# lh3/bwa

Hardware: AMD Instinct MI355X
Metric: Mreads/s (whole job) 2x150 bp vs GRCh38-scale index; SAM bit-identical to bwa mem (gate: `parity`).  `value` = the hot path (mem_align1_core of every read) on batches resident in HBM, as the bench contract times it; the SAM-producing FASTQ->SAM rate of the same build is `end_to_end_pe.value` (also i (higher is better)
Workload: dtype int32/u64 (integer DP + FM-index ranks); 1 GPU; 500000 pairs of 2x150 bp (mates interleaved) per GPU per step vs seeded synthetic 3100 Mbp genome (GRCh38 stand-in, seq_len 6.2e+09; BASELINE configs[2] layout); reads_per_gpu=1000000, read_len=150, layout=pe, sa_intv=1, occ_block_bytes=32, batches_in_flight=3

## Files before the change

bwa_amd/api.py:

```python
from __future__ import annotations

import ctypes as C
import os

import numpy as np

try:
    import torch
except Exception:
    torch = None

from .structs import ALN_DTYPE, ALNREG_DTYPE, PAIR_DTYPE, PESTAT_DTYPE, PESTAT_INFO_DTYPE, PRIMARY_DTYPE, RESCUE_DTYPE, SAMPE_DTYPE, MemOpt, PeOut, SamIn, SamOut

HERE = os.path.dirname(os.path.abspath(__file__))
DEFAULT_LIB = os.path.join(HERE, "csrc", "libbwagpu.so")

INTV3_DTYPE = np.dtype([("x0", "<u8"), ("x2", "<u8"), ("info", "<u8")])
GCHAIN_DTYPE = np.dtype([("n_seeds", "<i4"), ("rid", "<i4"), ("w", "<i4"), ("kept", "<i4"), ("is_alt", "<i4"),
                         ("frac_rep", "<f4"), ("pos", "<i8")])
GSEED_DTYPE = np.dtype([("rbeg", "<i8"), ("qbeg", "<i4"), ("len", "<i4"), ("score", "<i4"), ("_pad", "<i4")])
assert GCHAIN_DTYPE.itemsize == 32 and GSEED_DTYPE.itemsize == 24


MATESW_DTYPE = np.dtype([("read", "<i4"), ("r", "<i4"), ("anchor_rb", "<i8"), ("anchor_rid", "<i4"), ("score", "<i4"), ("te", "<i4"), ("qe", "<i4"),
# ... 7 lines not shown
SORT_KEY_DTYPE = np.dtype([("a", "<i8"), ("b", "<i4"), ("c", "<i4")])
assert SORT_KEY_DTYPE.itemsize == 16


class Stats(C.Structure):
    _fields_ = [(n, C.c_int64) for n in (
        "n_reads", "n_bases", "n_intv", "n_seeds", "n_chains", "n_regs_raw", "n_regs", "n_occ_blocks", "n_lf_steps",
        "n_ext_calls", "n_ext_cells", "n_glb_calls", "n_glb_cells", "ref_bases", "n_sw_calls", "n_sw_cells")] + [
        (n, C.c_float) for n in ("ms_seed", "ms_sa", "ms_chain", "ms_seedsw", "ms_extend", "ms_dedup", "ms_total")] + [
        ("n_retries", C.c_int32), ("ms_publish", C.c_float), ("n_tab_lookups", C.c_int64), ("n_bt_nodes", C.c_int64), ("n_chain_recs", C.c_int64),
        ("n_chain_deferred", C.c_int64), ("n_ext_fast", C.c_int64), ("n_chain_deferred2", C.c_int64),
        ("ms_pack", C.c_float), ("ms_download_copy", C.c_float), ("ms_cigar_kernels", C.c_float), ("ms_cigar_copy", C.c_float),
        ("n_cig_cells", C.c_int64), ("n_cig_dp", C.c_int64), ("retry_mask", C.c_int32), ("reserved_", C.c_int32)]

    def as_dict(self):
        return {n: getattr(self, n) for n, _ in self._fields_ if n != "reserved_"}


EXPORTS = [
    "bwagpu_create", "bwagpu_create_from_files", "bwagpu_destroy", "bwagpu_strerror", "bwagpu_last_error", "bwagpu_version",
    "bwagpu_index_info", "bwagpu_densify_sa", "bwagpu_set_stats", "bwagpu_get_stats", "bwagpu_align_bseq", "bwagpu_align_flat",
    "bwagpu_free", "bwagpu_batch_upload", "bwagpu_batch_run", "bwagpu_batch_download", "bwagpu_set_taps", "bwagpu_tap_intervals",
    "bwagpu_tap_chains", "bwagpu_tap_regs_raw", "bwagpu_index_buffers", "bwagpu_index_export", "bwagpu_clone", "bwagpu_index_ready",
    "bwagpu_batch_cigars", "bwagpu_batch_cigar_ops", "bwagpu_debug_phase", "bwagpu_batch_matesw", "bwagpu_clone_to_device", "bwagpu_index_build", "bwagpu_built_free", "bwagpu_abi_sizes", "bwagpu_debug_prof", "bwagpu_debug_hist", "bwagpu_debug_seed_x2", "bwagpu_debug_chain_hist", "bwagpu_debug_dp", "bwagpu_debug_sort", "bwagpu_debug_sort_limits", "bwagpu_set_cigar_filter", "bwagpu_batch_reserve", "bwagpu_batch_footprint", "bwagpu_mem_info",
    "bwagpu_batch_primary", "bwagpu_primary_flat", "bwagpu_primary_limits", "bwagpu_batch_pair", "bwagpu_pair_flat", "bwagpu_pair_limits", "bwagpu_batch_rescue", "bwagpu_rescue_flat", "bwagpu_rescue_limits",
    "bwagpu_batch_pestat", "bwagpu_pestat_flat", "bwagpu_batch_pestat_hist", "bwagpu_pestat_finish", "bwagpu_pestat_limits",
    "bwagpu_batch_alns", "bwagpu_alns_flat", "bwagpu_alns_limits", "bwagpu_aln_size",
    "bwagpu_cigars_flat", "bwagpu_cigar_limits", "bwagpu_dedup_flat", "bwagpu_dedup_limits", "bwagpu_ext_limits", "bwagpu_seed_limits",
    "bwagpu_batch_sampe", "bwagpu_sampe_flat", "bwagpu_sampe_limits", "bwagpu_sampe_size",
    "bwagpu_set_contig_names", "bwagpu_batch_sam", "bwagpu_sam_flat", "bwagpu_sam_limits",
    "bwagpu_trim", "bwagpu_set_option", "bwagpu_get_option", "bwagpu_set_default_option", "bwagpu_clear_default_options", "bwagpu_option_name",
]


class IndexDesc(C.Structure):
    _fields_ = [("bwt", C.c_void_p), ("bwt_size", C.c_uint64), ("primary", C.c_uint64), ("L2", C.c_uint64 * 5), ("seq_len", C.c_uint64),
                ("sa", C.c_void_p), ("n_sa", C.c_uint64), ("sa_intv", C.c_int), ("pac", C.c_void_p), ("l_pac", C.c_int64),
                ("n_seqs", C.c_int32), ("ctg_offset", C.c_void_p), ("ctg_len", C.c_void_p), ("ctg_is_alt", C.c_void_p)]


class BwaGpuError(RuntimeError):
    pass


def load_library(path: str | None = None) -> C.CDLL:
    path = path or DEFAULT_LIB
    if not os.path.exists(path):
# ... 763 lines not shown
```

bwa_amd/csrc/bwagpu.hip:

```cpp
#include <hip/hip_runtime.h>
#include <stdio.h>
#include <stdlib.h>
#include <string.h>
#include <math.h>
#include <algorithm>
#include <atomic>
#include <map>
#include <memory>
#include <mutex>
#include <string>
#include <vector>
#include <chrono>

#include "bwagpu_config.h"
#include "dev_common.h"
#include "dev_fm.h"
#include "dev_sort.h"
#include "dev_seed.h"
#include "dev_chain.h"
#include "dev_chainw.h"
#include "dev_ext.h"
#include "dev_extw.h"
#include "dev_extp.h"
#include "dev_dedup.h"
// ... 187 lines not shown
{
	if (b.ensure(bytes ? bytes : 16)) { h->err = "hipMalloc failed"; return BWAGPU_ENOMEM; }
	if (bytes) HIPCHK(h, hipMemcpy(b.p, src, bytes, hipMemcpyHostToDevice));
	return 0;
}

namespace {
std::mutex g_cfg_m;
std::map<std::string, long long> g_cfg_defaults;
}
static bool option_in_range(const BwagpuConfig &c, const long long *f, long long value)
{
	auto in = [&](long long lo, long long hi) { return value >= lo && value <= hi; };
	if (f == &c.ext_occ) return value == 4 || value == 6;
	if (f == &c.seed_mrg) return value == -1 || value == 0 || value == 2;
	if (f == &c.share) return in(-1, 100);
	if (f == &c.seed_task_stack || f == &c.seed_p2_cap || f == &c.mem_cap || f == &c.seed_grid || f == &c.cig_ops_cap || f == &c.idx_desc_max_mb || f == &c.pri_log_cap || f == &c.pair_tab_cap) return in(0, 0x3fffffff);
	if (f == &c.seed_budget || f == &c.dedup_heavy) return in(-1, 0x3fffffff);
	if (f == &c.dedup_stage || f == &c.dedup_big || f == &c.dedup_net) return in(-1, 1024);
	if (f == &c.seed_lds_ent) return in(-1, 16);
	if (f == &c.dedup_ring) return value == 0 || (in(256, 4096) && (value & (value - 1)) == 0);
	if (f == &c.cigl_mib) return in(0, 1 << 20);
	if (f == &c.cig_tiers || f == &c.chain_regs) return in(0, 2);
	if (f == &c.chain_flt_lds) return in(0, CW_FLT_LDS);
	if (f == &c.ptab_m) return in(0, PTAB_MAX);
	if (f == &c.occ32_sb_shift) return in(8, 32);
	return true;
}
static void init_config(BwagpuConfig &c)
{
	c = BwagpuConfig();
	const BwagpuConfig dflt;
	c.from_env();
#define X(name, d) if (!option_in_range(c, &c.name, c.name)) { fprintf(stderr, "[W::bwagpu] BWAGPU_%s=%lld is out of range: ignored\n", #name, c.name); c.name = dflt.name; }
	BWAGPU_OPTION_LIST(X)
#undef X
	std::lock_guard<std::mutex> l(g_cfg_m);
	for (auto &kv : g_cfg_defaults) if (long long *f = c.field(kv.first.c_str())) *f = kv.second;
	g_results.on = c.pinned_results; g_results.min_kb = c.pinned_min_kb < 0 ? 0 : c.pinned_min_kb; g_results.cap_mb = c.pinned_cap_mb < 0 ? 0 : c.pinned_cap_mb; g_results.inited = true;
}
extern "C" int bwagpu_set_default_option(const char *key, long long value)
{
	BwagpuConfig probe;
	const long long *f = probe.field(key);
	if (!f || !option_in_range(probe, f, value)) return BWAGPU_EINVAL;
	std::lock_guard<std::mutex> l(g_cfg_m);
// ... 37 lines not shown
__global__ void __launch_bounds__(256) k_ptab_level(DevIndex ix, u64 *tab, int j)
{
	const u64 n = (u64)1 << (2 * j);
	for (u64 c = (u64)blockIdx.x * blockDim.x + threadIdx.x; c < n; c += (u64)gridDim.x * blockDim.x) {
		BiIntv out;
		if (j == 1) fm_init(ix, (int)c, out);
		else {
			const u64 *pe = tab + ((((u64)1 << (2 * (j - 1))) - 4) / 3 + (c >> 2)) * 3;
			BiIntv par; par.x0 = pe[0]; par.x1 = pe[1]; par.x2 = pe[2]; par.info = 0;
			fm_extend1(ix, par, 3 - (int)(c & 3), 0, out);
		}
		u64 *e = tab + ((n - 4) / 3 + c) * 3;
		e[0] = out.x0; e[1] = out.x1; e[2] = out.x2;
	}
}

__global__ void __launch_bounds__(256) k_ptab_records(const u64 *tab, uint4 *rec, int m)
{
	const u64 n = ((u64)1 << (2 * m)) * (u64)m;
	for (u64 t = (u64)blockIdx.x * blockDim.x + threadIdx.x; t < n; t += (u64)gridDim.x * blockDim.x) {
		const u64 w = t / (u64)m; const int j = (int)(t % (u64)m) + 1;
		const u64 *e = tab + ((((u64)1 << (2 * j)) - 4) / 3 + (w >> (2 * (m - j)))) * 3;
		BiIntv v; v.x0 = e[0]; v.x1 = e[1]; v.x2 = e[2]; v.info = 0;
		rec[t] = SeedStack::pack(v);
	}
}

DEVFN void occ32_start_counts(const DevIndex &ix, u64 j, u64 cnt[4])
{
	const uint4 *src = ix.bwt + (j >> 1) * 4;
	const uint4 c01 = src[0], c23 = src[1];
	cnt[0] = (u64)c01.y << 32 | c01.x; cnt[1] = (u64)c01.w << 32 | c01.z; cnt[2] = (u64)c23.y << 32 | c23.x; cnt[3] = (u64)c23.w << 32 | c23.z;
	if (j & 1) {
		const uint4 w0 = src[2];
		u32 c1 = 0, c2 = 0, c3 = 0;
		count_pair(w0.x, w0.y, 32, c1, c2, c3); count_pair(w0.z, w0.w, 32, c1, c2, c3);
		cnt[0] += 64 - c1 - c2 - c3; cnt[1] += c1; cnt[2] += c2; cnt[3] += c3;
	}
}
__global__ void __launch_bounds__(256) k_occ32_sb(DevIndex ix, u64 *sb, u64 n_sb, u64 n_new, int sh )
{
	for (u64 s = (u64)blockIdx.x * blockDim.x + threadIdx.x; s < n_sb; s += (u64)gridDim.x * blockDim.x) {
		u64 cnt[4] = { 0, 0, 0, 0 };
		if ((s << sh) < n_new) occ32_start_counts(ix, s << sh, cnt);
		for (int k = 0; k < 4; ++k) sb[s * 4 + k] = cnt[k];
	}
// ... 345 lines not shown
	if (ctg_is_alt) memcpy(ctg_is_alt, h->h_ctg_alt.data(), (size_t)h->n_seqs * 4);
	return BWAGPU_OK;
}

extern "C" int bwagpu_index_info(const bwagpu_t *h, int64_t *l_pac, int32_t *n_seqs, uint64_t *seq_len, int *sa_intv)
{
	if (!h) return BWAGPU_EINVAL;
	if (l_pac) *l_pac = h->l_pac;
	if (n_seqs) *n_seqs = h->n_seqs;
	if (seq_len) *seq_len = h->seq_len;
	if (sa_intv) *sa_intv = h->sa_intv;
	return BWAGPU_OK;
}

extern "C" int bwagpu_debug_phase(const bwagpu_t *h) { return h ? h->phase : -1; }
extern "C" int bwagpu_debug_prof(bwagpu_t *h, unsigned long long out[16])
{
	if (!h || !out || !h->d_ctr.p) return BWAGPU_EINVAL;
	Counters c;
	if (hipMemcpy(&c, h->d_ctr.p, sizeof c, hipMemcpyDeviceToHost) != hipSuccess) return BWAGPU_EHIP;
	for (int i = 0; i < 16; ++i) out[i] = c.prof[i];
	out[8] = c.n_vr_ovf + c.prof[8];
	out[0] = c.n_heavy; out[1] = c.n_p2_tasks;
	return BWAGPU_OK;
}

extern "C" int bwagpu_debug_seed_x2(bwagpu_t *h, unsigned long long out[8])
{
	if (!h || !out || !h->d_ctr.p) return BWAGPU_EINVAL;
	Counters c;
	if (hipMemcpy(&c, h->d_ctr.p, sizeof c, hipMemcpyDeviceToHost) != hipSuccess) return BWAGPU_EHIP;
	for (int i = 0; i < 8; ++i) out[i] = c.seed_x2[i];
	return BWAGPU_OK;
}
extern "C" int bwagpu_debug_hist(bwagpu_t *h, unsigned long long out[256])
{
	if (!h || !out || !h->d_ctr.p) return BWAGPU_EINVAL;
	Counters c;
	if (hipMemcpy(&c, h->d_ctr.p, sizeof c, hipMemcpyDeviceToHost) != hipSuccess) return BWAGPU_EHIP;
	for (int i = 0; i < 64; ++i) out[i] = c.seed_hist[i];
	for (int i = 0; i < 96; ++i) { out[64 + i] = c.wave_hist[0][i]; out[160 + i] = c.wave_hist[1][i]; }
	return BWAGPU_OK;
}
extern "C" int bwagpu_debug_chain_hist(bwagpu_t *h, unsigned long long out[192])
{
	if (!h || !out || !h->d_ctr.p) return BWAGPU_EINVAL;
// ... 360 lines not shown
		Batch B; memset(&B, 0, sizeof B);
		B.n_reads = n; B.max_len = h->max_len; B.stats = h->stats_on;
		B.seq = h->d_seq.as<u8>(); B.seq_nib = h->d_seq_nib.as<u64>(); B.off = h->d_off.as<i64>(); B.ctr = h->d_ctr.as<Counters>();
		B.tmp_intv = h->d_tmp_intv.as<BiIntv>(); B.mem_cap = h->mem_cap;
		B.rd_words = h->rd_words; B.seq_2b = h->d_seq_2b.as<u32>(); B.seq_flags = h->d_seq_flags.as<u8>();
		const int lane_lds = SEED_LANE_LDS, ent_max = SEED_LDS_ENT;
		const int lds_ent_dflt = h->rd_words ? ((lane_lds - 4 * h->rd_words) / 16 < ent_max ? (lane_lds - 4 * h->rd_words) / 16 : ent_max) : ent_max;
		B.seed_lds_ent = (h->seq_len < ((u64)1 << 37) && h->max_len < 65536) ? (cfg.seed_lds_ent >= 0 ? (int)cfg.seed_lds_ent : lds_ent_dflt) : 0;
		h->seed_lds_run = B.seed_lds_ent;
		if (((size_t)(B.seed_lds_ent ? B.seed_lds_ent : 1) * 16 + (size_t)B.rd_words * 4) * BLOCK > 65536) B.rd_words = 0;
		B.intv_n = h->d_intv_n.as<i32>(); B.intv_off = h->d_intv_off.as<i64>(); B.intv = h->d_intv.as<Intv3>();
		B.seed_n = h->d_seed_n.as<i32>(); B.seed_off = h->d_seed_off.as<i64>(); B.slot_cap = h->slot_cap;
		B.slot_pos = h->d_slot_pos.as<u64>(); B.slot_qbeg = h->d_slot_qbeg.as<i32>(); B.slot_len = h->d_slot_len.as<i32>(); B.slot_rid = h->d_slot_rid.as<i32>(); B.slot_blob = h->d_slot_blob.as<u8>();
		B.chain_n = h->d_chain_n.as<i32>(); B.node_off = h->d_node_off.as<i64>(); B.nodes = h->d_nodes.as<i32>(); B.node_cap = h->node_cap;
		B.reg_off = h->d_reg_off.as<i64>(); B.reg_cap_r = h->d_reg_cap_r.as<i32>(); B.reg_n_raw = h->d_reg_n_raw.as<i32>(); B.reg_n = h->d_reg_n.as<i32>();
		B.regs = h->d_regs.as<bwagpu_alnreg_t>(); B.reg_cap = h->reg_cap;
		B.regs_raw = h->taps_on ? h->d_regs_raw.as<bwagpu_alnreg_t>() : nullptr;
		B.dp_h = h->d_dp_h.as<i32>(); B.dp_e = h->d_dp_e.as<i32>(); B.dp_waves = dp_wave_count(h, n_threads);
		B.seedsw_minhsp = h->d_minhsp.as<i32>();
		B.order = h->d_order.as<i32>(); B.bin_cnt = h->d_bin_cnt.as<u32>(); B.seed_w = h->d_seed_w.as<i32>(); B.seed_order = nullptr;
		B.seed_prio = cfg.seed_prio != 0;
		B.ext_blk = cfg.ext_blk != 0;
		B.seed_no_virt = cfg.seed_no_virt != 0;
		B.seed_pass3_inline = cfg.seed_pass3_inline != 0;
		B.task_step = opt->min_seed_len; B.n_vreads = n_vreads; B.vr_ovf_run = 0; B.vr_room = 0; B.seed_stack_cap = 0; B.intv_n3 = nullptr;
		if (seed_tasks) { B.vr_first = h->d_vr_tab.as<i32>(); B.vr_ovf = h->d_vr_ovf.as<i32>(); B.intv_n3 = h->d_intv_n3.as<i32>(); }
		B.task_tpr = 0; B.p2_tasks = nullptr; B.p2_cap = 0; B.heavy_list = nullptr; B.seed_budget = 0;
		if (heavy_tasks) {
			const i64 p2_cap = cfg.seed_p2_cap > 0 ? cfg.seed_p2_cap * (i64)h->p2_factor : (i64)((double)n * .5 * h->p2_factor) + 4096;
			B.heavy_list = h->d_heavy.as<i32>(); B.seed_budget = seed_budget;
			if (h->d_p2_tasks.ensure((size_t)p2_cap * 8)) { h->err = "hipMalloc failed (seeding tasks)"; return BWAGPU_ENOMEM; }
			B.intv_n3 = h->d_intv_n3.as<i32>(); B.p2_tasks = h->d_p2_tasks.as<i64>(); B.p2_cap = p2_cap;
		}
		int seed_mrg = (cfg.seed_mrg >= 0 ? cfg.seed_mrg : 2) ? 2 : 0;
		if (!idx_in_desc) seed_mrg = 0;
		B.seq_nib_bytes = (((u64)h->n_bases + 15) / 16) * 8;
		dim3 grid(n_threads / BLOCK), block(BLOCK);
		HIPCHK(h, hipEventRecord(h->ev[0], h->stream));
		if (dbg_sync) { hipError_t e_ = hipStreamSynchronize(h->stream); fprintf(stderr, "[bwagpu] attempt %d: %s done (%s)\n", attempt, "start", hipGetErrorString(e_)); }
		if (!B.seed_pass3_inline) {
			if (h->ix.occ32 != nullptr && seed_mrg) hipLaunchKernelGGL((k_seed3<1, true>), grid, block, 0, h->stream, h->ix, *opt, B);
			else if (h->ix.occ32 != nullptr) hipLaunchKernelGGL(k_seed3<1>, grid, block, 0, h->stream, h->ix, *opt, B);
			else hipLaunchKernelGGL(k_seed3<0>, grid, block, 0, h->stream, h->ix, *opt, B);
			if (!cfg.seed_input_order) {
				i32 *keep = B.order; B.order = h->d_seed_order.as<i32>();
				if (int rc2 = order_reads(h, B, B.seed_w)) return rc2;
// ... 2070 lines not shown
```

bwa_amd/csrc/bwagpu_config.h:

```cpp
#pragma once
#include <stdlib.h>
#include <string.h>
#include <ctype.h>
#include <string>

#define BWAGPU_OPTION_LIST(X) \
	X(occ32,             1)     \
	X(occ32_sb_shift,    32)    \
	X(ptab_m,            10)    \
	X(idx_desc_max_mb,   0)     \
	X(seed_mrg,          -1)    \
	X(seed_tasks,        -1)    \
	X(seed_budget,       -1)    \
	X(seed_p2_cap,       0)     \
	X(seed_task_stack,   0)     \
	X(publish_blk,       -1)    \
	X(seedsw_lds,        -1)    \
	X(dedup_blk,         -1)    \
	X(seed_lds_ent,      -1)    \
	X(seed_rd_lds,       1)     \
	X(seed_no_virt,      0)     \
	X(seed_prio,         1)     \
	X(seed_input_order,  0)     \
	X(seed_pass3_inline, 0)     \
	X(seed_grid,         0)     \
	X(share,             -1)    \
	X(ext_pack,          0)     \
	X(ext_blk,           -1)    \
	X(ext_occ,           6)     \
	X(chain_regs,        2)     \
	X(chain_flt_lds,     256)   \
	X(dedup_heavy,       -1)    \
	X(dedup_stage,       -1)    \
	X(dedup_big,         -1)    \
	X(dedup_net,         -1)    \
	X(dedup_prio,        1)     \
	X(dedup_wave,        0)     \
	X(dedup_ring,        0)     \
	X(mem_cap,           0)     \
	X(cig_tiers,         2)     \
	X(cig_ops_cap,       0)     \
	X(cig_long,          1)     \
	X(cigl_mib,          32768) \
	X(pri_log_cap,       0)     \
// ... 29 lines not shown
```

bwa_amd/csrc/dev_common.h:

```cpp
#pragma once
#include <hip/hip_runtime.h>
#include <stdint.h>
#include "../../include/bwagpu.h"

typedef uint64_t u64;
typedef int64_t i64;
typedef uint32_t u32;
typedef int32_t i32;
typedef uint8_t u8;

#define DEVFN __device__ __forceinline__
#ifndef DEV_KEEP
#define DEV_KEEP(v) asm volatile("" : "+v"(v))
#endif
typedef __amdgpu_buffer_rsrc_t BufRsrc;

struct DevIndex {
	const uint4 *bwt;
	u64 primary, L2[5], seq_len;
	const u64 *sa;
	u64 sa_mask;
	int sa_shift;
	const u8 *pac;
	i64 l_pac;
// ... 93 lines not shown
	RegionView v;
	v.chain = (ChainRec*)b; v.kinfo = (int4*)(b + (size_t)64 * n); v.cchain = (bwagpu_chain_t*)(b + (size_t)80 * n);
	v.cseed = (bwagpu_seed_t*)(b + (size_t)112 * n); v.srt = (u64*)(b + (size_t)136 * n);
	v.next = (i32*)(b + (size_t)144 * n); v.ord = (i32*)(b + (size_t)148 * n); v.kept = (i32*)(b + (size_t)152 * n);
	return v;
}

struct Batch {
	int n_reads;
	int max_len;
	int stats;
	const u8 *seq;
	u64 *seq_nib;
	u64 seq_nib_bytes;
	const i64 *off;
	u32 *seq_2b;
	u8 *seq_flags;
	int rd_words;
	Counters *ctr;
	BiIntv *tmp_intv;
	int seed_stack_cap;
	int seed_lds_ent;
	int seed_no_virt;
	int mem_cap;
	i32 *seed_w;
	const i32 *seed_order;
	i32 *intv_n;
	i64 *intv_off;
	Intv3 *intv;
	i32 *seed_n;
	i64 *seed_off;
	i64 slot_cap;
	u64 *slot_pos;
	i32 *slot_qbeg, *slot_len;
	i32 *slot_rid;
	u8 *slot_blob;
	i32 *chain_n;
	int task_step, n_vreads;
	int task_tpr;
	i32 *heavy_list;
	i32 *dd_list;
	int dd_heavy_min, dd_stage_cap;
	int dd_net;
	int dd_prio;
	i32 *dd_form;
	int seed_budget;
// ... 40 lines not shown
```

bwa_amd/csrc/dev_seed.h:

```cpp
#pragma once
#include "dev_fm.h"
#include "dev_sort.h"

#define PTAB_MAX 12
#define SEED_CAND_BITS 64

struct SeedEmit {
	Intv3 *intv; int r, n, cap; bool overflow;
	int min_seed_len;
	i32 *shared_n;
	DEVFN Intv3 *mem() const { return intv + (size_t)r * (size_t)cap; }
	int split_len, base; u64 split_width, cand;
	DEVFN void add(u64 x0, u64 x2, int start, int end) {
		if (end - start < min_seed_len) return;
		Intv3 v; v.x0 = x0; v.x2 = x2; v.info = (u64)start << 32 | (u32)end;
		if (shared_n) {
			const int k = atomicAdd(&shared_n[r], 1);
			if (k >= cap) overflow = true; else mem()[k] = v;
			return;
		}
		if (n == cap) { overflow = true; return; }
		if (end - start >= split_len && x2 <= split_width && n - base < SEED_CAND_BITS) cand |= 1ull << (n - base);
		mem()[n++] = v;
	}
// ... 13 lines not shown
	const u32 *rd;
	int rd_on;
	const u8 *raw; const i64 *off;
	u64 min_intv, last_x2;
	int sx, i, n0, nprev, nc, j, c, ret, last_start;
	int lo;
	bool any;
	BiIntv ik;
	u32 code;
	u32 smask, srem, snew;
	int ncl;
	int top;
	int slot;
	SeedEmit em;
};

struct SeedStack {
	uint4 *lds_base;
	BiIntv *glob_base; int glob_cap;
	DEVFN uint4 *lds_col() const { return lds_base + threadIdx.x; }
	DEVFN BiIntv *glob_col() const { return glob_base + (size_t)(blockIdx.x * blockDim.x + threadIdx.x) * (size_t)glob_cap + PTAB_MAX; }
	int stride, n_lds;
	int virt_m;
	DEVFN void push_fw(SeedLane &L, const BiIntv &v) const {
		const int len = (int)v.info - L.sx;
		if (len < virt_m) L.smask |= 1u << (len - 1); else push(L, v);
	}
	static DEVFN uint4 pack(const BiIntv &v) {
		uint4 w;
		w.x = (u32)v.x0; w.y = (u32)v.x1; w.z = (u32)v.x2;
		w.w = (u32)(v.x0 >> 32) | (u32)(v.x1 >> 32) << 5 | (u32)(v.x2 >> 32) << 10 | (u32)v.info << 16;
		return w;
	}
	static DEVFN BiIntv unpack(const uint4 &w) {
		BiIntv v;
		v.x0 = (u64)(w.w & 31) << 32 | w.x; v.x1 = (u64)(w.w >> 5 & 31) << 32 | w.y; v.x2 = (u64)(w.w >> 10 & 31) << 32 | w.z;
		v.info = w.w >> 16;
		return v;
	}
	DEVFN void push(SeedLane &L, const BiIntv &v) const {
		if (n_lds == 0) glob_col()[L.n0] = v;
		else {
			if (L.n0 >= n_lds) ((uint4*)glob_col())[L.n0 - n_lds] = lds_col()[L.slot * stride];
			lds_col()[L.slot * stride] = pack(v);
			L.slot = L.slot + 1 == n_lds ? 0 : L.slot + 1;
		}
// ... 39 lines not shown
		for (int k = 0; k < 4; ++k)
			for (int b = 0; b < 4; ++b) {
				u32 c = d[k] >> (8 * b) & 255;
				o |= (u64)(c > 3 ? 4 : c) << ((k * 4 + b) * 4);
			}
		B.seq_nib[w] = o;
	}
}

__global__ void __launch_bounds__(256) k_pack_reads2b(Batch B)
{
	const u64 total = (u64)B.n_reads * (u64)B.rd_words;
	for (u64 t = (u64)blockIdx.x * blockDim.x + threadIdx.x; t < total; t += (u64)gridDim.x * blockDim.x) {
		const int r = (int)(t / (u32)B.rd_words), j = (int)(t % (u32)B.rd_words);
		const i64 b0 = B.off[r] + 16 * (i64)j, left = B.off[r + 1] - b0;
		u32 o = 0; bool any_n = false;
		for (int k = 0; k < 16 && k < left; ++k) {
			const u32 c = B.seq[b0 + k];
			if (c > 3) any_n = true; else o |= c << (2 * k);
		}
		B.seq_2b[t] = o;
		if (any_n) B.seq_flags[r] = 1;
	}
}

DEVFN void smem_finish(SeedLane &L) { if (L.pass == 1) { L.x = L.ret; L.st = SS_PASS1; } else L.st = SS_PASS2; }

DEVFN void bwd_begin_row(SeedLane &L, const SeedStack &S, const u64 *nib, int m)
{
	for (;;) {
		if (L.i < L.lo) { smem_finish(L); return; }
		L.c = L.i < 0 ? -1 : seed_q(L, nib, L.i);
		if (L.c > 3) L.c = -1;
		L.j = 0; L.nc = 0; L.ncl = 0; L.last_x2 = 0; L.srem = L.smask; L.snew = 0;
		if (L.c >= 0) { if (m > 0) L.code = (u32)L.c << (2 * (m - 1)) | L.code >> 2; L.st = SS_BWD; return; }
		if (!L.any || L.i + 1 < L.last_start) {
			if (L.nprev > 0) { BiIntv p = S.load(L, 0); L.em.add(p.x0, p.x2, L.i + 1, (int)p.info); }
			L.any = true; L.last_start = L.i + 1;
		}
		smem_finish(L);
		return;
	}
}

DEVFN void fwd_finish(SeedLane &L, const SeedStack &S, const u64 *nib, int m)
{
// ... 8 lines not shown
{
	out = SeedStack::unpack(ix.ptab[(u64)w * (u32)ix.ptab_m + (u32)(j - 1)]);
}

struct SeedBufs { Occ32Bufs occ; BufRsrc ptab, stk, nib; };
template <bool WIN = false> DEVFN int ext_one_trip(const DevIndex &ix, const SeedBufs &bf, bool ext, bool blocks, const BiIntv &src, int c, int back, int tl, u32 code, BiIntv &ok, u32 pf_off, uint4 &pf, u32 win_off = BUF_OOB, u64 *win = nullptr)
{
	const Occ32Pos pp = occ32_pos(ix, src, back);
	Occ32Data od;
	uint4 te = buf_load16(bf.ptab, ext && !blocks ? (code * (u32)ix.ptab_m + (u32)(tl - 1)) << 4 : BUF_OOB);
	occ32_issue(ix, bf.occ, blocks, pp, c, od);
	pf = buf_load16(bf.stk, pf_off);
	uint2 wv = make_uint2(0, 0);
	if (WIN) { wv = buf_load8(bf.nib, win_off); DEV_KEEP(wv.x); DEV_KEEP(wv.y); *win = (u64)wv.y << 32 | wv.x; }
	occ32_keep(od); dev_keep(te); dev_keep(pf);
	int nb = 0;
	if (ext) {
		if (!blocks) ok = SeedStack::unpack(te);
		else nb = occ32_finish(ix, src, c, back, pp, od, ok);
	}
	return nb;
}

DEVFN u32 window_code(SeedLane &L, const u64 *nib, int x, int m)
{
	u32 rc = 0;
	for (int k = 0; k < m; ++k) { const int g = x + k; rc = rc << 2 | (u32)((g < L.len ? seed_q(L, nib, g) : 0) & 3); }
	return rc;
}


DEVFN void smem_start(const DevIndex &ix, SeedLane &L, const SeedStack &S, const u64 *nib, int x, u64 min_intv, int pass)
{
	L.pass = pass; L.sx = x; L.min_intv = min_intv < 1 ? 1 : min_intv;
	const int c0 = seed_q(L, nib, x);
	if (c0 > 3) { L.ret = x + 1; smem_finish(L); return; }
	fm_init(ix, c0, L.ik); L.ik.info = (u64)(x + 1);
	L.i = x + 1; L.n0 = 0; L.slot = 0; L.smask = 0;
	L.code = window_code(L, nib, x, ix.ptab_m);
	if (L.i >= L.len || seed_q(L, nib, L.i) > 3) {
		S.push_fw(L, L.ik); L.ret = (int)L.ik.info;
		fwd_finish(L, S, nib, ix.ptab_m);
	} else L.st = SS_FWD;
}

__global__ void __launch_bounds__(256) k_publish(bwagpu_opt_t opt, Batch B)
{
	u64 nintv = 0;
	for (int r = blockIdx.x * blockDim.x + threadIdx.x; r < B.n_reads; r += gridDim.x * blockDim.x) {
		int n = B.intv_n[r];
		if (n > B.mem_cap) { atomicOr(&B.ctr->overflow, 16ull); B.intv_n[r] = 0; n = 0; }
		B.intv_off[r] = (i64)r * B.mem_cap;
		B.seed_n[r] = 0; B.seed_off[r] = 0; B.node_off[r] = 0;
		if (n == 0) continue;
		Intv3 *iv = B.intv + (size_t)r * B.mem_cap;
		dev_introsort(iv, n, IntvInfoLess());
		i64 ns = 0;
		for (int i = 0; i < n; ++i) {
			const u64 x2 = iv[i].x2;
			u64 step = x2 > (u64)opt.max_occ ? x2 / opt.max_occ : 1;
			u64 cnt = (x2 + step - 1) / step;
			ns += (i64)(cnt < (u64)opt.max_occ ? cnt : (u64)opt.max_occ);
// ... 111 lines not shown
					i64 k = 0;
					for (u32 c = 0; c < cnt; ++c, k += step, ++s) { B.slot_pos[s] = p.x0 + (u64)k; B.slot_qbeg[s] = qb; B.slot_len[s] = sl; }
				}
				base += (u32)s_bcast[0];
				__syncthreads();
			}
		}
		__syncthreads();
	}
	if (B.stats && tid == 0) atomicAdd(&B.ctr->n_intv, (unsigned long long)nintv);
}

template<bool RD, bool STATS, int BLK, int OCC, int MRG = 0, int LR = 0>
__global__ void __launch_bounds__(256, OCC) k_seed(DevIndex ix, bwagpu_opt_t opt, Batch B)
{
	HIP_DYNAMIC_SHARED(uint4, seed_lds)
	const int cap = B.seed_stack_cap > 0 ? B.seed_stack_cap : B.max_len + 1 + PTAB_MAX;
	const int split_len = (int)(opt.min_seed_len * opt.split_factor + .499);
	SeedLane L;
	SeedStack S;
	S.lds_base = seed_lds; S.stride = blockDim.x; S.n_lds = B.seed_lds_ent;
	S.glob_base = B.tmp_intv; S.glob_cap = cap;
	S.virt_m = (ix.ptab_m >= 2 && opt.min_seed_len > ix.ptab_m && !B.seed_no_virt) ? ix.ptab_m : 0;
	L.smask = L.srem = L.snew = 0; L.ncl = 0;
	L.em.intv = B.intv; L.em.r = -1; L.em.cap = B.mem_cap; L.em.min_seed_len = opt.min_seed_len;
	L.em.split_len = split_len; L.em.split_width = (u64)opt.split_width; L.em.cand = 0; L.em.base = 0; L.em.shared_n = LR == 1 ? B.intv_n : nullptr;
	L.lo = -1;
	int vr_task = -1, vr_run = 0;
	const unsigned long long n_tasks = LR == 1 ? (B.vr_ovf_run ? B.ctr->n_vr_ovf : B.task_tpr > 0 ? B.ctr->n_heavy * (unsigned long long)B.task_tpr : (unsigned long long)B.n_vreads)
									 : LR == 3 ? (B.ctr->n_p2_tasks < (unsigned long long)B.p2_cap ? B.ctr->n_p2_tasks : (unsigned long long)B.p2_cap) : 0;
	if (LR == 3) L.em.shared_n = B.intv_n;
	int p2_entry = 0;
	L.st = SS_FETCH; L.len = 0; L.qoff = 0; L.win = 0; L.win_w = ~0u; L.win2 = 0; L.win2_w = ~0u;
	u32 *rd_lds = (u32*)(seed_lds + (size_t)(B.seed_lds_ent ? B.seed_lds_ent : 1) * blockDim.x);
	L.rd = rd_lds; L.rd_on = 0; L.raw = B.seq; L.off = B.off;
	const u64 *nib = RD ? nullptr : B.seq_nib;
	u32 nblk = 0, ntab = 0;
	int pool_base = 0, pool_cnt = 0, pool_r = 0;
	int deferred = 0;
	u32 n_iter = 0, n_slow = 0, n_ext_lanes = 0, n_deep = 0, n_deep_l = 0, n_pf_l = 0, n_win_l = 0;
	u32 n_done_l = 0, n_wait_l = 0, n_slowrun_l = 0, n_first_done = 0;
	u32 n_x2[6] = { 0, 0, 0, 0, 0, 0 }; bool run_f = false, run_b = false;
	u32 my_iter = 0;
	uint4 pf = make_uint4(0, 0, 0, 0);
	SeedBufs bf;
	if (MRG && BLK == 1) {
// ... 141 lines not shown
				case SS_PASS3:
					while (L.x < L.len && seed_q(L, nib, L.x) > 3) ++L.x;
					if (L.x >= L.len) L.st = SS_FINAL;
					else {
						const int c0 = seed_q(L, nib, L.x);
						fm_init(ix, c0, L.ik); L.sx = L.x; L.i = L.x + 1;
						L.code = window_code(L, nib, L.x, ix.ptab_m);
						if (L.i >= L.len) { L.x = L.len; }
						else if (seed_q(L, nib, L.i) > 3) { L.x = L.i + 1; }
						else L.st = SS_STRAT;
					}
					break;
				default: break;
				}
			}
		}
		const int st = L.st;
		if (STATS) n_ext_lanes += (u32)__popcll(__ballot(st == SS_FWD || st == SS_BWD || st == SS_STRAT));
		if (STATS && __ballot(st == SS_BWD && L.j >= S.n_lds && L.j < L.nprev)) ++n_deep;
		const bool ext = st == SS_FWD || st == SS_BWD || st == SS_STRAT;
		BiIntv ok, src, p;
		p.x0 = p.x1 = p.x2 = p.info = 0;
		const int back = st == SS_BWD;
		bool short_ent = false;
		int cb = 0, tl = 0;
		ok.x0 = ok.x1 = ok.x2 = ok.info = 0; src = ok;
		if (ext) {
			if (back) {
				if (L.j < L.nprev) {
					if (STATS && L.j >= S.n_lds) { ++n_deep_l; if (MRG == 2 && pf.w != 0) ++n_pf_l; }
					if (MRG == 2 && pf.w != 0) p = SeedStack::unpack(pf); else p = S.load(L, L.j);
				} else {
					const int len = 32 - __clz((int)L.srem);
					L.srem &= ~(1u << (len - 1));
					p.x0 = p.x1 = p.x2 = 0; p.info = (u64)(L.i + 1 + len); short_ent = true;
				}
			}
			src.x0 = back ? p.x0 : L.ik.x0; src.x1 = back ? p.x1 : L.ik.x1; src.x2 = back ? p.x2 : L.ik.x2; src.info = 0;
			const int qi = back ? 0 : seed_q(L, nib, L.i);
			cb = back ? L.c : 3 - qi;
			tl = back ? (int)p.info - L.i : L.i - L.sx + 1;
		}
		const bool blocks = ext && tl > ix.ptab_m;
		if (MRG && BLK == 1) {
			u32 pf_off = BUF_OOB;
			if (MRG == 2 && back && !short_ent && S.n_lds && L.j + 1 < L.nprev && L.j + 1 >= S.n_lds)
				pf_off = ((u32)threadIdx.x * (u32)S.glob_cap + PTAB_MAX) * (u32)sizeof(BiIntv) + (u32)(L.top - (L.j + 1)) * (u32)sizeof(uint4);
			u32 nb;
			if (MRG == 2 && !RD) {
				u32 win_off = BUF_OOB, ww = 0; u64 wnew = 0;
				const int want = back ? L.i - 1 : L.i + 1;
				if (ext && want >= 0 && want < L.len) {
					ww = (u32)((L.qoff + (u64)want) >> 4);
					if (ww != L.win_w && ww != L.win2_w) win_off = ww << 3;
				}
				nb = (u32)ext_one_trip<true>(ix, bf, ext, blocks, src, cb, back, tl, L.code, ok, pf_off, pf, win_off, &wnew);
				if (win_off != BUF_OOB && B.seq_nib_bytes <= BUF_MAX_BYTES) { L.win2 = wnew; L.win2_w = ww; if (STATS) ++n_win_l; }
			} else nb = (u32)ext_one_trip(ix, bf, ext, blocks, src, cb, back, tl, L.code, ok, pf_off, pf);
			if (STATS && ext) { if (blocks) nblk += nb; else ++ntab; }
		}
		if (STATS && ext && blocks) {
			const bool one = src.x2 == 1;
			++n_x2[back ? 1 : 0]; if (one) ++n_x2[back ? 3 : 2];
			if (one && !(back ? run_b : run_f)) ++n_x2[back ? 5 : 4];
			if (back) run_b = one; else run_f = one;
		}
		if (ext) {
			if (MRG && BLK == 1) ;
			else if (!blocks) { ptab_load(ix, tl, L.code, ok); if (STATS) ++ntab; }
			else { const u32 nb = fm_extend1<BLK>(ix, src, cb, back, ok); if (STATS) nblk += nb; }
			if (LR == 1 && st == SS_FWD && L.n0 >= B.vr_room) {
				const unsigned long long k = atomicAdd(&B.ctr->n_vr_ovf, 1ull);
				B.vr_ovf[k] = vr_task;
				L.st = SS_FINAL;
			} else
			if (st == SS_FWD) {
				bool stop = false;
				if (ok.x2 != L.ik.x2) {
					S.push_fw(L, L.ik); L.ret = (int)L.ik.info;
					if (ok.x2 < L.min_intv) stop = true;
				}
				if (!stop) {
					ok.info = (u64)(L.i + 1); L.ik = ok; ++L.i;
					if (L.i >= L.len || seed_q(L, nib, L.i) > 3) { S.push_fw(L, L.ik); L.ret = (int)L.ik.info; stop = true; }
				}
				if (stop) fwd_finish(L, S, nib, ix.ptab_m);
			} else if (st == SS_BWD) {
				if (ok.x2 < L.min_intv) {
					if (L.nc == 0 && (!L.any || L.i + 1 < L.last_start)) {
						L.em.add(p.x0, p.x2, L.i + 1, (int)p.info); L.any = true; L.last_start = L.i + 1;
					}
				} else if (L.nc == 0 || ok.x2 != L.last_x2) {
					ok.info = p.info;
					const int nl = (int)p.info - L.i;
					if (nl < S.virt_m) L.snew |= 1u << (nl - 1);
					else { S.store(L, L.ncl, ok); ++L.ncl; }
					++L.nc; L.last_x2 = ok.x2;
				}
				if (!short_ent) ++L.j;
				if (L.j >= L.nprev && L.srem == 0) {
					if (L.nc == 0) smem_finish(L);
					else { L.nprev = L.ncl; L.smask = L.snew; --L.i; bwd_begin_row(L, S, nib, ix.ptab_m); }
				}
			} else {
				if (ok.x2 < opt.max_mem_intv && L.i - L.sx >= opt.min_seed_len) {
					if (ok.x2 > 0) L.em.add(ok.x0, ok.x2, L.sx, L.i + 1);
					L.x = L.i + 1; L.st = SS_PASS3;
				} else {
					L.ik = ok; ++L.i;
					if (L.i >= L.len) { L.x = L.len; L.st = SS_PASS3; }
					else if (seed_q(L, nib, L.i) > 3) { L.x = L.i + 1; L.st = SS_PASS3; }
				}
			}
		}
	}
	if (STATS) {
		atomicAdd(&B.ctr->occ_blocks, (unsigned long long)nblk); atomicAdd(&B.ctr->tab_lookups, (unsigned long long)ntab);
		for (int k = 0; k < 6; ++k) atomicAdd(&B.ctr->seed_x2[k], (unsigned long long)n_x2[k]);
		atomicAdd(&B.ctr->prof[9], (unsigned long long)n_win_l); atomicAdd(&B.ctr->prof[10], (unsigned long long)n_deep_l); atomicAdd(&B.ctr->prof[11], (unsigned long long)n_pf_l);
		if ((threadIdx.x & 63) == 0) { atomicAdd(&B.ctr->prof[12], (unsigned long long)n_deep); atomicAdd(&B.ctr->prof[13], (unsigned long long)n_iter); atomicAdd(&B.ctr->prof[14], (unsigned long long)n_slow); atomicAdd(&B.ctr->prof[15], (unsigned long long)n_ext_lanes);
// ... 13 lines not shown
		const Intv3 *iv = B.intv + (size_t)r * (size_t)B.mem_cap;
		for (int e = n3; e < n; ++e) {
			const Intv3 p = iv[e];
			const int start = (int)(p.info >> 32), end = (int)(u32)p.info;
			if (end - start < split_len || p.x2 > (u64)opt.split_width) continue;
			const unsigned long long t = atomicAdd(&B.ctr->n_p2_tasks, 1ull);
			if ((long long)t < B.p2_cap) B.p2_tasks[t] = (i64)r << 32 | (u32)e; else atomicOr(&B.ctr->overflow, 32ull);
		}
	}
}

template <int BLK, bool MRG = false> __global__ void __launch_bounds__(256, 3) k_seed3(DevIndex ix, bwagpu_opt_t opt, Batch B)
{
	SeedLane L;
	L.em.cap = B.mem_cap; L.em.min_seed_len = opt.min_seed_len; L.em.intv = B.intv; L.em.r = -1; L.em.n = 0; L.em.overflow = false;
	L.em.split_len = 0x7fffffff; L.em.split_width = 0; L.em.cand = 0; L.em.base = 0; L.em.shared_n = nullptr;
	L.len = 0; L.qoff = 0; L.win = 0; L.win_w = ~0u; L.win2 = 0; L.win2_w = ~0u; L.x = 0; L.sx = 0; L.i = 0; L.code = 0; L.rd = nullptr; L.rd_on = 0; L.raw = nullptr; L.off = nullptr;
	L.ik.x0 = L.ik.x1 = L.ik.x2 = L.ik.info = 0;
	const u64 *nib = B.seq_nib;
	const int lane = threadIdx.x & 63;
	enum { T_FETCH = 0, T_START, T_EXT, T_DONE };
	int st = T_FETCH, pool_base = 0, pool_cnt = 0;
	u32 nblk = 0, ntab = 0, weight = 0;
	SeedBufs bf;
	if (MRG && BLK == 1) { bf.occ = occ32_bufs(ix); bf.ptab = buf_rsrc(ix.ptab, ix.ptab_bytes); bf.stk = buf_rsrc(nullptr, 0); bf.nib = bf.stk; }
	while (__ballot(st != T_DONE)) {
		const u64 wm = __ballot(st == T_FETCH);
		if (wm) {
			if (pool_cnt == 0) {
				const int first = __ffsll((unsigned long long)__ballot(1)) - 1;
				const unsigned long long old = atomicAdd(&B.ctr->next_read3, lane == first ? 64ull : 0ull);
				pool_base = __shfl((int)old, first); pool_cnt = 64;
			}
			const int rank = __popcll(wm & ((1ull << lane) - 1));
			if (st == T_FETCH && rank < pool_cnt) {
				const int r = pool_base + rank;
				if (r >= B.n_reads) st = T_DONE;
				else {
					L.em.r = r; L.qoff = (u64)B.off[r]; L.len = (int)(B.off[r + 1] - B.off[r]);
					L.em.n = 0; L.em.overflow = false;
					B.intv_n[r] = 0; B.seed_w[r] = 0; weight = 0;
					if (B.intv_n3) B.intv_n3[r] = 0;
					if (L.len >= opt.min_seed_len && opt.max_mem_intv > 0) { L.x = 0; st = T_START; }
				}
			}
			const int took = __popcll(wm) < pool_cnt ? __popcll(wm) : pool_cnt;
			pool_base += took; pool_cnt -= took;
		}
		if (st == T_START) {
			while (L.x < L.len && seed_q(L, nib, L.x) > 3) ++L.x;
			if (L.x >= L.len) {
				if (L.em.overflow) atomicOr(&B.ctr->overflow, 16ull); else { B.intv_n[L.em.r] = L.em.n; if (B.intv_n3) B.intv_n3[L.em.r] = L.em.n; }
				B.seed_w[L.em.r] = (i32)(weight > 0x3fffffffu ? 0x3fffffffu : weight);
				st = T_FETCH;
			} else {
				fm_init(ix, seed_q(L, nib, L.x), L.ik); L.sx = L.x; L.i = L.x + 1;
				L.code = window_code(L, nib, L.x, ix.ptab_m);
				if (L.i >= L.len) L.x = L.len;
				else if (seed_q(L, nib, L.i) > 3) L.x = L.i + 1;
				else st = T_EXT;
			}
		}
		const bool ext = st == T_EXT;
		const int tl = L.i - L.sx + 1;
		const bool blocks = ext && tl > ix.ptab_m;
		const int cb = blocks ? 3 - seed_q(L, nib, L.i) : 0;
		BiIntv ok; ok.x0 = ok.x1 = ok.x2 = ok.info = 0;
		if (MRG && BLK == 1) {
			uint4 none;
			BiIntv srcv = L.ik; if (!ext) srcv.x0 = srcv.x1 = srcv.x2 = 0;
			const int nb = ext_one_trip(ix, bf, ext, blocks, srcv, cb, 0, tl, L.code, ok, BUF_OOB, none);
			if (ext) { if (blocks) nblk += nb; else ++ntab; }
		}
		if (ext) {
			if (MRG && BLK == 1) ;
			else if (!blocks) { ptab_load(ix, tl, L.code, ok); ++ntab; }
			else nblk += fm_extend1<BLK>(ix, L.ik, cb, 0, ok);
			if (tl == opt.min_seed_len) weight += (u32)(ok.x2 > 65535 ? 65535 : ok.x2);
			if (ok.x2 < opt.max_mem_intv && L.i - L.sx >= opt.min_seed_len) {
				if (ok.x2 > 0) L.em.add(ok.x0, ok.x2, L.sx, L.i + 1);
// ... 39 lines not shown
```

include/bwagpu.h:

```cpp
#ifndef BWAGPU_H
#define BWAGPU_H

#include <stdint.h>
#include <stddef.h>

#ifdef __cplusplus
extern "C" {
#endif

#define BWAGPU_OK        0
#define BWAGPU_ENODEV   -1
#define BWAGPU_EINVAL   -2
#define BWAGPU_ENOMEM   -3
#define BWAGPU_EIO      -4
#define BWAGPU_EHIP     -5
#define BWAGPU_EUNSUP   -6

typedef struct bwagpu_s bwagpu_t;

typedef struct {
	int a, b;
	int o_del, e_del;
	int o_ins, e_ins;
	int pen_unpaired;
// ... 106 lines not shown
	float ms_seed, ms_sa, ms_chain, ms_seedsw, ms_extend, ms_dedup, ms_total;
	int32_t n_retries;
	float ms_publish;
	int64_t n_tab_lookups;
	int64_t n_bt_nodes;
	int64_t n_chain_recs;
	int64_t n_chain_deferred;
	int64_t n_ext_fast;
	int64_t n_chain_deferred2;
	float ms_pack;
	float ms_download_copy;
	float ms_cigar_kernels;
	float ms_cigar_copy;
	int64_t n_cig_cells;
	int64_t n_cig_dp;
	int32_t retry_mask;
	int32_t reserved_;
} bwagpu_stats_t;

int bwagpu_debug_phase(const bwagpu_t *h);
int bwagpu_debug_prof(bwagpu_t *h, unsigned long long out[16]);
int bwagpu_debug_hist(bwagpu_t *h, unsigned long long out[256]);
int bwagpu_debug_seed_x2(bwagpu_t *h, unsigned long long out[8]);
int bwagpu_debug_chain_hist(bwagpu_t *h, unsigned long long out[192]);

typedef struct {
	int32_t q_off, q_len, t_off, t_len;
	int32_t w;
	int32_t h0;
	int32_t end_bonus;
	int32_t flags;
} bwagpu_dp_case_t;
int bwagpu_debug_dp(bwagpu_t *h, const bwagpu_opt_t *opt, int kind, int n_cases, const bwagpu_dp_case_t *cases, const uint8_t *seqs, int64_t n_seq_bytes, int32_t *out);

typedef struct { int64_t a; int32_t b, c; } bwagpu_sort_key_t;
void bwagpu_debug_sort_limits(int32_t out[8]);
int bwagpu_debug_sort(bwagpu_t *h, int kind, int n_cases, const bwagpu_sort_key_t *keys, const int64_t *off, int dd_net, int par_cap, int chain_flt_lds, int32_t *perm, int32_t *status);

int bwagpu_batch_cigars(bwagpu_t *h, const bwagpu_opt_t *opt, bwagpu_cigar_t **out, int64_t *n_out);
int bwagpu_set_cigar_filter(bwagpu_t *h, int enable);
int bwagpu_batch_cigar_ops(bwagpu_t *h, uint32_t **ops, int64_t *n_ops);
int bwagpu_cigars_flat(bwagpu_t *h, const bwagpu_opt_t *opt, int n_reads, const uint8_t *seqs, const int64_t *seq_off, const int32_t *counts, const bwagpu_alnreg_t *regs,
					   bwagpu_cigar_t **cigs, int64_t *n_cigs, uint32_t **ops, int64_t *n_ops);
void bwagpu_cigar_limits(int32_t out[10]);
int bwagpu_dedup_flat(bwagpu_t *h, const bwagpu_opt_t *opt, int n_reads, const uint8_t *seqs, const int64_t *seq_off, const int32_t *counts, const bwagpu_alnreg_t *regs,
					  int32_t *counts_out, bwagpu_alnreg_t **regs_out, int64_t *n_out, int32_t *form);
// ... 309 lines not shown
```

Baseline: 11.58 Mreads/s.

## Jump SMEM forward extension across prefix-table window using precomputed interval-change masks

Prefix-table records now carry a bitmask showing at which prefix lengths the SA interval size changes. When the first m bases are unambiguous, forward extension jumps straight to the end of the window instead of stepping one base at a time, and rebuilds the per-length push mask from the stored bits. On the backward pass, the first short entry derives the surviving short intervals in one bit-manipulation step instead of iterating. This saves FM-index steps per seed start, at the cost of more complex state handling and a fallback when the jumped interval drops below min_intv.

```diff
diff --git a/bwa_amd/api.py b/bwa_amd/api.py
--- a/bwa_amd/api.py
+++ b/bwa_amd/api.py
@@ -53,7 +53,7 @@
     "bwagpu_index_info", "bwagpu_densify_sa", "bwagpu_set_stats", "bwagpu_get_stats", "bwagpu_align_bseq", "bwagpu_align_flat",
     "bwagpu_free", "bwagpu_batch_upload", "bwagpu_batch_run", "bwagpu_batch_download", "bwagpu_set_taps", "bwagpu_tap_intervals",
     "bwagpu_tap_chains", "bwagpu_tap_regs_raw", "bwagpu_index_buffers", "bwagpu_index_export", "bwagpu_clone", "bwagpu_index_ready",
-    "bwagpu_batch_cigars", "bwagpu_batch_cigar_ops", "bwagpu_debug_phase", "bwagpu_batch_matesw", "bwagpu_clone_to_device", "bwagpu_index_build", "bwagpu_built_free", "bwagpu_abi_sizes", "bwagpu_debug_prof", "bwagpu_debug_hist", "bwagpu_debug_seed_x2", "bwagpu_debug_chain_hist", "bwagpu_debug_dp", "bwagpu_debug_sort", "bwagpu_debug_sort_limits", "bwagpu_set_cigar_filter", "bwagpu_batch_reserve", "bwagpu_batch_footprint", "bwagpu_mem_info",
+    "bwagpu_batch_cigars", "bwagpu_batch_cigar_ops", "bwagpu_debug_phase", "bwagpu_batch_matesw", "bwagpu_clone_to_device", "bwagpu_index_build", "bwagpu_built_free", "bwagpu_abi_sizes", "bwagpu_debug_prof", "bwagpu_debug_hist", "bwagpu_debug_seed_x2", "bwagpu_debug_ptab", "bwagpu_debug_chain_hist", "bwagpu_debug_dp", "bwagpu_debug_sort", "bwagpu_debug_sort_limits", "bwagpu_set_cigar_filter", "bwagpu_batch_reserve", "bwagpu_batch_footprint", "bwagpu_mem_info",
     "bwagpu_batch_primary", "bwagpu_primary_flat", "bwagpu_primary_limits", "bwagpu_batch_pair", "bwagpu_pair_flat", "bwagpu_pair_limits", "bwagpu_batch_rescue", "bwagpu_rescue_flat", "bwagpu_rescue_limits",
     "bwagpu_batch_pestat", "bwagpu_pestat_flat", "bwagpu_batch_pestat_hist", "bwagpu_pestat_finish", "bwagpu_pestat_limits",
     "bwagpu_batch_alns", "bwagpu_alns_flat", "bwagpu_alns_limits", "bwagpu_aln_size",
diff --git a/bwa_amd/csrc/bwagpu.hip b/bwa_amd/csrc/bwagpu.hip
--- a/bwa_amd/csrc/bwagpu.hip
+++ b/bwa_amd/csrc/bwagpu.hip
@@ -233,6 +233,7 @@
 	if (f == &c.dedup_ring) return value == 0 || (in(256, 4096) && (value & (value - 1)) == 0);
 	if (f == &c.cigl_mib) return in(0, 1 << 20);
 	if (f == &c.cig_tiers || f == &c.chain_regs) return in(0, 2);
+	if (f == &c.seed_jump) return in(-1, 3);
 	if (f == &c.chain_flt_lds) return in(0, CW_FLT_LDS);
 	if (f == &c.ptab_m) return in(0, PTAB_MAX);
 	if (f == &c.occ32_sb_shift) return in(8, 32);
@@ -316,6 +317,12 @@
 		const u64 w = t / (u64)m; const int j = (int)(t % (u64)m) + 1;
 		const u64 *e = tab + ((((u64)1 << (2 * j)) - 4) / 3 + (w >> (2 * (m - j)))) * 3;
 		BiIntv v; v.x0 = e[0]; v.x1 = e[1]; v.x2 = e[2]; v.info = 0;
+		u64 deeper = v.x2;
+		for (int k = j - 1; k >= 1; --k) {
+			const u64 x2 = tab[((((u64)1 << (2 * k)) - 4) / 3 + (w >> (2 * (m - k)))) * 3 + 2];
+			if (x2 != deeper) v.info |= (u64)1 << (k - 1);
+			deeper = x2;
+		}
 		rec[t] = SeedStack::pack(v);
 	}
 }
@@ -707,6 +714,14 @@
 	for (int i = 0; i < 16; ++i) out[i] = c.prof[i];
 	out[8] = c.n_vr_ovf + c.prof[8];
 	out[0] = c.n_heavy; out[1] = c.n_p2_tasks;
+	return BWAGPU_OK;
+}
+
+extern "C" int bwagpu_debug_ptab(bwagpu_t *h, int32_t *m, uint64_t *bytes, void *out)
+{
+	if (!h || !m || !bytes) return BWAGPU_EINVAL;
+	*m = h->ix.ptab ? h->ix.ptab_m : 0; *bytes = h->ix.ptab ? h->ix.ptab_bytes : 0;
+	if (out && *bytes && hipMemcpy(out, h->ix.ptab, *bytes, hipMemcpyDeviceToHost) != hipSuccess) return BWAGPU_EHIP;
 	return BWAGPU_OK;
 }
 
@@ -1113,6 +1128,7 @@
 		B.seed_prio = cfg.seed_prio != 0;
 		B.ext_blk = cfg.ext_blk != 0;
 		B.seed_no_virt = cfg.seed_no_virt != 0;
+		B.seed_jump = cfg.seed_jump < 0 ? 3 : (int)cfg.seed_jump;
 		B.seed_pass3_inline = cfg.seed_pass3_inline != 0;
 		B.task_step = opt->min_seed_len; B.n_vreads = n_vreads; B.vr_ovf_run = 0; B.vr_room = 0; B.seed_stack_cap = 0; B.intv_n3 = nullptr;
 		if (seed_tasks) { B.vr_first = h->d_vr_tab.as<i32>(); B.vr_ovf = h->d_vr_ovf.as<i32>(); B.intv_n3 = h->d_intv_n3.as<i32>(); }
diff --git a/bwa_amd/csrc/bwagpu_config.h b/bwa_amd/csrc/bwagpu_config.h
--- a/bwa_amd/csrc/bwagpu_config.h
+++ b/bwa_amd/csrc/bwagpu_config.h
@@ -20,6 +20,7 @@
 	X(seed_lds_ent,      -1)    \
 	X(seed_rd_lds,       1)     \
 	X(seed_no_virt,      0)     \
+	X(seed_jump,         -1)    \
 	X(seed_prio,         1)     \
 	X(seed_input_order,  0)     \
 	X(seed_pass3_inline, 0)     \
diff --git a/bwa_amd/csrc/dev_common.h b/bwa_amd/csrc/dev_common.h
--- a/bwa_amd/csrc/dev_common.h
+++ b/bwa_amd/csrc/dev_common.h
@@ -139,6 +139,7 @@
 	int seed_stack_cap;
 	int seed_lds_ent;
 	int seed_no_virt;
+	int seed_jump;
 	int mem_cap;
 	i32 *seed_w;
 	const i32 *seed_order;
diff --git a/bwa_amd/csrc/dev_seed.h b/bwa_amd/csrc/dev_seed.h
--- a/bwa_amd/csrc/dev_seed.h
+++ b/bwa_amd/csrc/dev_seed.h
@@ -59,6 +59,7 @@
 	DEVFN BiIntv *glob_col() const { return glob_base + (size_t)(blockIdx.x * blockDim.x + threadIdx.x) * (size_t)glob_cap + PTAB_MAX; }
 	int stride, n_lds;
 	int virt_m;
+	int jump;
 	DEVFN void push_fw(SeedLane &L, const BiIntv &v) const {
 		const int len = (int)v.info - L.sx;
 		if (len < virt_m) L.smask |= 1u << (len - 1); else push(L, v);
@@ -144,6 +145,16 @@
 		B.seq_2b[t] = o;
 		if (any_n) B.seq_flags[r] = 1;
 	}
+}
+
+DEVFN u32 rev32(u32 x)
+{
+#ifdef __clang__
+	return __builtin_bitreverse32(x);
+#else
+	x = (x >> 1 & 0x55555555u) | (x & 0x55555555u) << 1; x = (x >> 2 & 0x33333333u) | (x & 0x33333333u) << 2; x = (x >> 4 & 0x0f0f0f0fu) | (x & 0x0f0f0f0fu) << 4;
+	return __builtin_bswap32(x);
+#endif
 }
 
 DEVFN void smem_finish(SeedLane &L) { if (L.pass == 1) { L.x = L.ret; L.st = SS_PASS1; } else L.st = SS_PASS2; }
@@ -198,10 +209,17 @@
 	return nb;
 }
 
-DEVFN u32 window_code(SeedLane &L, const u64 *nib, int x, int m)
-{
-	u32 rc = 0;
-	for (int k = 0; k < m; ++k) { const int g = x + k; rc = rc << 2 | (u32)((g < L.len ? seed_q(L, nib, g) : 0) & 3); }
+#define SEED_JUMP_FLAG 0x80000000u
+DEVFN u32 window_code(SeedLane &L, const u64 *nib, int x, int m, bool *partial = nullptr)
+{
+	u32 rc = 0; bool part = false;
+	for (int k = 0; k < m; ++k) {
+		const int g = x + k;
+		const int c = g < L.len ? seed_q(L, nib, g) : 4;
+		if (c > 3) part = true;
+		rc = rc << 2 | (u32)(c & 3);
+	}
+	if (partial) *partial = part;
 	return rc;
 }
 
@@ -213,7 +231,11 @@
 	if (c0 > 3) { L.ret = x + 1; smem_finish(L); return; }
 	fm_init(ix, c0, L.ik); L.ik.info = (u64)(x + 1);
 	L.i = x + 1; L.n0 = 0; L.slot = 0; L.smask = 0;
-	L.code = window_code(L, nib, x, ix.ptab_m);
+	bool partial;
+	L.code = window_code(L, nib, x, ix.ptab_m, &partial);
+	if ((S.jump & 1) && !partial) {
+		L.i = x + S.virt_m - 1; L.smask = SEED_JUMP_FLAG; L.st = SS_FWD;
+	} else
 	if (L.i >= L.len || seed_q(L, nib, L.i) > 3) {
 		S.push_fw(L, L.ik); L.ret = (int)L.ik.info;
 		fwd_finish(L, S, nib, ix.ptab_m);
@@ -371,6 +393,7 @@
 	S.lds_base = seed_lds; S.stride = blockDim.x; S.n_lds = B.seed_lds_ent;
 	S.glob_base = B.tmp_intv; S.glob_cap = cap;
 	S.virt_m = (ix.ptab_m >= 2 && opt.min_seed_len > ix.ptab_m && !B.seed_no_virt) ? ix.ptab_m : 0;
+	S.jump = S.virt_m > 0 ? B.seed_jump : 0;
 	L.smask = L.srem = L.snew = 0; L.ncl = 0;
 	L.em.intv = B.intv; L.em.r = -1; L.em.cap = B.mem_cap; L.em.min_seed_len = opt.min_seed_len;
 	L.em.split_len = split_len; L.em.split_width = (u64)opt.split_width; L.em.cand = 0; L.em.base = 0; L.em.shared_n = LR == 1 ? B.intv_n : nullptr;
@@ -558,7 +581,7 @@
 		BiIntv ok, src, p;
 		p.x0 = p.x1 = p.x2 = p.info = 0;
 		const int back = st == SS_BWD;
-		bool short_ent = false;
+		bool short_ent = false, first_short = false;
 		int cb = 0, tl = 0;
 		ok.x0 = ok.x1 = ok.x2 = ok.info = 0; src = ok;
 		if (ext) {
@@ -568,6 +591,7 @@
 					if (MRG == 2 && pf.w != 0) p = SeedStack::unpack(pf); else p = S.load(L, L.j);
 				} else {
 					const int len = 32 - __clz((int)L.srem);
+					first_short = (S.jump & 2) && L.srem == L.smask;
 					L.srem &= ~(1u << (len - 1));
 					p.x0 = p.x1 = p.x2 = 0; p.info = (u64)(L.i + 1 + len); short_ent = true;
 				}
@@ -611,17 +635,23 @@
 				L.st = SS_FINAL;
 			} else
 			if (st == SS_FWD) {
-				bool stop = false;
-				if (ok.x2 != L.ik.x2) {
-					S.push_fw(L, L.ik); L.ret = (int)L.ik.info;
-					if (ok.x2 < L.min_intv) stop = true;
-				}
-				if (!stop) {
-					ok.info = (u64)(L.i + 1); L.ik = ok; ++L.i;
-					if (L.i >= L.len || seed_q(L, nib, L.i) > 3) { S.push_fw(L, L.ik); L.ret = (int)L.ik.info; stop = true; }
-				}
-				if (stop) fwd_finish(L, S, nib, ix.ptab_m);
+				const bool jumped = (L.smask & SEED_JUMP_FLAG) != 0;
+				if (jumped && ok.x2 < L.min_intv) { L.smask = 0; L.i = L.sx + 1; }
+				else {
+					bool stop = false;
+					if (jumped) L.smask = (u32)ok.info;
+					else if (ok.x2 != L.ik.x2) {
+						S.push_fw(L, L.ik); L.ret = (int)L.ik.info;
+						if (ok.x2 < L.min_intv) stop = true;
+					}
+					if (!stop) {
+						ok.info = (u64)(L.i + 1); L.ik = ok; ++L.i;
+						if (L.i >= L.len || seed_q(L, nib, L.i) > 3) { S.push_fw(L, L.ik); L.ret = (int)L.ik.info; stop = true; }
+					}
+					if (stop) fwd_finish(L, S, nib, ix.ptab_m);
+				}
 			} else if (st == SS_BWD) {
+				const u32 chg = (u32)ok.info;
 				if (ok.x2 < L.min_intv) {
 					if (L.nc == 0 && (!L.any || L.i + 1 < L.last_start)) {
 						L.em.add(p.x0, p.x2, L.i + 1, (int)p.info); L.any = true; L.last_start = L.i + 1;
@@ -632,6 +662,12 @@
 					if (nl < S.virt_m) L.snew |= 1u << (nl - 1);
 					else { S.store(L, L.ncl, ok); ++L.ncl; }
 					++L.nc; L.last_x2 = ok.x2;
+				}
+				if (first_short && L.srem && ok.x2 >= L.min_intv) {
+					const int b1 = (int)p.info - L.i - 2;
+					const u32 rs = rev32(L.srem), below = ~(rs | 0x80000000u >> b1), c2 = rev32((chg & ((2u << b1) - 1)) >> 1);
+					const u32 kept = rev32((((c2 & below) + below) | c2) & rs);
+					L.snew |= kept << 1; L.nc += __popc(kept); L.srem = 0;
 				}
 				if (!short_ent) ++L.j;
 				if (L.j >= L.nprev && L.srem == 0) {
@@ -691,6 +727,7 @@
 	enum { T_FETCH = 0, T_START, T_EXT, T_DONE };
 	int st = T_FETCH, pool_base = 0, pool_cnt = 0;
 	u32 nblk = 0, ntab = 0, weight = 0;
+	const bool jump = (B.seed_jump & 1) && ix.ptab_m >= 2 && ix.ptab_m <= opt.min_seed_len;
 	SeedBufs bf;
 	if (MRG && BLK == 1) { bf.occ = occ32_bufs(ix); bf.ptab = buf_rsrc(ix.ptab, ix.ptab_bytes); bf.stk = buf_rsrc(nullptr, 0); bf.nib = bf.stk; }
 	while (__ballot(st != T_DONE)) {
@@ -724,7 +761,10 @@
 				st = T_FETCH;
 			} else {
 				fm_init(ix, seed_q(L, nib, L.x), L.ik); L.sx = L.x; L.i = L.x + 1;
-				L.code = window_code(L, nib, L.x, ix.ptab_m);
+				bool partial;
+				L.code = window_code(L, nib, L.x, ix.ptab_m, &partial);
+				if (jump && !partial) { L.i = L.x + ix.ptab_m - 1; st = T_EXT; }
+				else
 				if (L.i >= L.len) L.x = L.len;
 				else if (seed_q(L, nib, L.i) > 3) L.x = L.i + 1;
 				else st = T_EXT;
diff --git a/include/bwagpu.h b/include/bwagpu.h
--- a/include/bwagpu.h
+++ b/include/bwagpu.h
@@ -152,6 +152,7 @@
 int bwagpu_debug_prof(bwagpu_t *h, unsigned long long out[16]);
 int bwagpu_debug_hist(bwagpu_t *h, unsigned long long out[256]);
 int bwagpu_debug_seed_x2(bwagpu_t *h, unsigned long long out[8]);
+int bwagpu_debug_ptab(bwagpu_t *h, int32_t *m, uint64_t *bytes, void *out);
 int bwagpu_debug_chain_hist(bwagpu_t *h, unsigned long long out[192]);
 
 typedef struct {
```

New measurement: 12.35 Mreads/s (median of 6 runs). 1.07x the previous value.
